# BenLangmead/bowtie2

Measured on NVIDIA H100. Metric: Mreads/s, higher is better.
Workload: dtype u64 popcount (FM rank) + s16x2 DPX (DP)

## Files before the change

bowtie2_b200/csrc/dp_kernels.cu:

```cuda
#include "fm_device.cuh"
#include "dp_device.cuh"

#define DP_NEG (-(1 << 28))
#define DP_BIG (1 << 20)

__host__ __device__ __forceinline__ size_t dp_smem_per_warp(int maxCol) { return ((size_t)maxCol * 7 + 16 + 15) & ~(size_t)15; }

__device__ __forceinline__ int dp_max(int a, int b) { return a > b ? a : b; }

template <int R>
__device__ __forceinline__ void dp_backtrace_all(const DpLaunch &L, const bt2g_scoring &sc, const bt2g_dp_problem &p, uint64_t w,
                                                 const uint8_t *rs, const uint8_t *rq, int rdlen, const uint8_t *refw,
                                                 uint8_t *codes, bt2g_dp_cand *cands, int ncand, bt2g_dp_summary *summ,
                                                 int lane, bool local) {
	const int rdgapo = sc.rdgap_const + sc.rdgap_linear, rdgape = sc.rdgap_linear;
	const int rfgapo = sc.rfgap_const + sc.rfgap_linear, rfgape = sc.rfgap_linear;
	int SQ = rdlen >> 4; if(SQ == 0) SQ = 1;
	bt2g_dp_aln *alns = L.alns + w * (uint64_t)L.maxAlns;
	uint8_t *ops = L.ops + w * (uint64_t)L.maxAlns * L.maxOps;
	int naln = 0, flags = 0;
	auto cell = [&](int rr, int cc) -> uint8_t * { int k = rr / R; return codes + ((size_t)(cc + k) * 32 + k) * R + (rr - k * R); };
	for(int ci = 0; ci < ncand; ci++) {
		int row = cands[ci].row, col = cands[ci].col;
		const int startRow = row;
// ... 79 lines not shown
			const int c = rdchar(row), refc = refw[col];
			const bool isN = c > 3 || refc > 3;
			ns += isN;
			const uint8_t op = (uint8_t)(((!isN && c == refc) ? BT2G_OP_MATCH : BT2G_OP_MM) | (refc << 2));
			if(!core) fail = true;
			else if(ns > p.nceil) fail = true;
			else {
				if(room && lane == 0 && nops < L.maxOps) o[nops] = op;
				nops++;
			}
		}
		const bool opOverflow = nops > L.maxOps;
		if(fail) { if(lane == 0) cands[ci].fate = BT2G_CAND_FAILED; continue; }
		if(lane == 0) cands[ci].fate = BT2G_CAND_SUCCEEDED;
		if(room) {
			int refns = 0;
			for(int k = col + lane; k <= origCol; k += 32) refns += refw[k] > 3;
			refns = __reduce_add_sync(0xffffffffu, refns);
			if(lane == 0) {
				bt2g_dp_aln &a = alns[naln];
				a.cand_idx = ci; a.score = cands[ci].score; a.ns = ns; a.gaps = gaps; a.col0 = col; a.row0 = row;
				a.trim_beg = trimBeg; a.trim_end = rdlen - 1 - startRow; a.nops = nops;
				a.refns = refns;
			}
			if(opOverflow) flags |= BT2G_DP_FLAG_OPS_OVERFLOW;
		} else {
			flags |= BT2G_DP_FLAG_ALN_OVERFLOW;
		}
		naln++;
	}
	if(lane == 0) { summ->naln = naln; summ->flags |= flags; }
}

template <typename Acc>
__device__ __forceinline__ void dp_backtrace_h(const DpLaunch &L, const bt2g_scoring &sc, const bt2g_dp_problem &p, uint64_t w,
                                               const uint8_t *rs, const uint8_t *rq, int rdlen, const uint8_t *refw,
                                               const Acc &cell, bt2g_dp_cand *cands, int ncand, bt2g_dp_summary *summ, int lane,
                                               const uint8_t *prof);

template <int R, bool HB = false, typename Acc = int>
__device__ __forceinline__ void dp_e2e_tail(const DpLaunch &L, const bt2g_scoring &sc, const bt2g_dp_problem &p, uint64_t w,
                                            const uint8_t *rs, const uint8_t *rq, int rdlen, int ncol, int32_t *lastH,
                                            uint16_t *candCol, const uint8_t *refw, uint8_t *codes, bt2g_dp_summary *summ, int lane,
                                            const Acc &hcell = Acc(), const uint8_t *prof = nullptr) {
	__syncwarp();
	int best = DP_NEG;
	for(int k = lane; k < ncol; k += 32) best = dp_max(best, lastH[k]);
#pragma unroll
	for(int o = 16; o > 0; o >>= 1) best = dp_max(best, __shfl_xor_sync(0xffffffffu, best, o));

	if(lane == 0) { summ->best = best; summ->flags = 0; summ->naln = 0; summ->ncand = 0; summ->found = 0; }
	if(best < p.minsc) return;
	bt2g_dp_cand *cands = L.cands + w * (uint64_t)L.maxCands;
	int totalCand = 0;
	for(int j0 = 0; j0 < ncol; j0 += 32) {
		const int j = j0 + lane;
		const int s = j < ncol ? lastH[j] : DP_NEG;
		const bool isC = j < ncol && s >= p.minsc;
		const uint32_t m = __ballot_sync(0xffffffffu, isC);
		if(isC) {
			const int k = totalCand + __popc(m & ((1u << lane) - 1u));
			lastH[k] = s; candCol[k] = (uint16_t)j;
		}
		totalCand += __popc(m);
		__syncwarp();
	}
	for(int a0 = 0; a0 < totalCand; a0 += 32) {
		const int a = a0 + lane;
		if(a < totalCand) {
			const int s = lastH[a];
			int rank = 0;
			for(int k = 0; k < totalCand; k++) {
				const int sk = lastH[k];
				rank += (sk > s) || (sk == s && k > a);
			}
			if(rank < L.maxCands) { cands[rank].score = s; cands[rank].col = candCol[a]; cands[rank].row = rdlen - 1; cands[rank].fate = 0; }
		}
	}
	const int ncand = totalCand < L.maxCands ? totalCand : L.maxCands;
	if(lane == 0) {
		summ->ncand = totalCand; summ->found = totalCand > 0;
		if(totalCand > L.maxCands) summ->flags |= BT2G_DP_FLAG_CAND_OVERFLOW;
	}
	__syncwarp();

	if constexpr(HB) dp_backtrace_h(L, sc, p, w, rs, rq, rdlen, refw, hcell, cands, ncand, summ, lane, prof);
	else dp_backtrace_all<R>(L, sc, p, w, rs, rq, rdlen, refw, codes, cands, ncand, summ, lane, false);
}

template <typename OFF, int R>
__global__ void __launch_bounds__(128) k_dp_e2e(DevIndex<OFF> ix, bt2g_scoring sc, DpLaunch L) {
	extern __shared__ uint8_t smem[];
	const int warpInBlock = threadIdx.x >> 5, lane = threadIdx.x & 31;
	const uint64_t slot = blockIdx.x * (uint64_t)(blockDim.x >> 5) + warpInBlock;
	const uint64_t nSlots = (uint64_t)gridDim.x * (blockDim.x >> 5);
	const uint64_t nProb = L.nDev ? (uint64_t)*L.nDev : L.n;
	const size_t perWarp = dp_smem_per_warp(L.maxCol);
	int32_t *lastH = reinterpret_cast<int32_t *>(smem + (size_t)warpInBlock * perWarp);
	uint16_t *candCol = reinterpret_cast<uint16_t *>(lastH + L.maxCol);
	uint8_t *refw = reinterpret_cast<uint8_t *>(candCol + L.maxCol);
	uint8_t *codes = L.codes + slot * L.codeStride;
	const int rdgapo = sc.rdgap_const + sc.rdgap_linear, rdgape = sc.rdgap_linear;
	const int rfgapo = sc.rfgap_const + sc.rfgap_linear, rfgape = sc.rfgap_linear;

	for(uint64_t w = slot; w < nProb; w += nSlots) {
		const bt2g_dp_problem p = L.probs[w];
		const uint8_t *rs = L.seq + L.roff[p.read_idx];
		const uint8_t *rq = L.qual + L.roff[p.read_idx];
		const int rdlen = (int)(L.roff[p.read_idx + 1] - L.roff[p.read_idx]);
		const int ncol = (int)(p.refr - p.refl + 1);
		bt2g_dp_summary *summ = L.summ + w;
		__syncwarp();
		if(ncol <= 0 || ncol > L.maxCol || rdlen > 32 * R || rdlen <= 0) {
			if(lane == 0) { summ->found = 0; summ->best = DP_NEG; summ->ncand = 0; summ->naln = 0; summ->flags = BT2G_DP_FLAG_BADSHAPE; }
			continue;
		}
		for(int k = lane; k < ncol; k += 32) refw[k] = (uint8_t)ref_base<OFF>(ix, p.tidx, p.refl + k);
		__syncwarp();

		int rc[R], mmpN[R], npnN[R], rfo[R], rfe[R], rdo[R];
// ... 607 lines not shown
						if(!TOP && OFFDOM && lo + t0 + SG - 1 >= bLast) {
							uint32_t s = botH | botF | prevInH;
#pragma unroll
							for(int r = 0; r < RPL; r++) s |= Hleft[r] | Earr[r];
							if(!__any_sync(0xffffffffu, t0 + SG - 1 - lane < lim && s != 0u)) return t0 + SG < nsteps ? t0 + SG : nsteps;
						}
					}
					return nsteps;
				};
				nst = b == 0 ? sweep(DpBool<true>()) : sweep(DpBool<false>());
			}
			if(lane == 0) {
				reinterpret_cast<uint32_t *>(hb[0])[b] = (uint32_t)lo | ((uint32_t)nst << 16);
				reinterpret_cast<uint32_t *>(hb[1])[b] = (uint32_t)lo | ((uint32_t)nst << 16);
			}
			off += (uint32_t)nst * 32 * RPL;
			plo = lo; phi = lo + nst - 32;
			if(phi > ncolMax - 1) phi = ncolMax - 1;
			__syncwarp();
		}
	}
}

struct DpHbBlocks {
	uint8_t *hb; const uint2 *tab;
	__device__ __forceinline__ uint8_t *operator()(int rr, int cc) const {
		const int k = (rr % DP_BLK_ROWS) / DP_BLOCK_RPL;
		const uint2 e = tab[rr / DP_BLK_ROWS];
		const int st = cc - (int)(e.x & 0xffffu) + k;
		return (st >= k && st < (int)(e.x >> 16)) ? hb + e.y + ((size_t)st * 32 + k) * DP_BLOCK_RPL + rr % DP_BLOCK_RPL : nullptr;
	}
};

#define DP_TAIL_SMEM_PER_WARP(maxCol, R) (dp_smem_per_warp(maxCol) + DP_PROF_BYTES(R) + DP_BLK_MAX * sizeof(uint2))

template <typename OFF, int R>
__global__ void __launch_bounds__(256) k_dp_tail_h(DevIndex<OFF> ix, bt2g_scoring sc, DpLaunch L, uint64_t chunkStart, uint64_t chunkMax,
                                                   uint32_t *next) {
	extern __shared__ uint8_t smem[];
	const int warpInBlock = threadIdx.x >> 5, lane = threadIdx.x & 31;
	const uint64_t nAll = L.nDev ? (uint64_t)*L.nDev : L.n;
	if(chunkStart >= nAll) return;
	const uint64_t nProb = (nAll - chunkStart < chunkMax) ? nAll - chunkStart : chunkMax;
	const size_t perWarp = DP_TAIL_SMEM_PER_WARP(L.maxCol, R);
	int32_t *lastH = reinterpret_cast<int32_t *>(smem + (size_t)warpInBlock * perWarp);
	uint16_t *candCol = reinterpret_cast<uint16_t *>(lastH + L.maxCol);
	uint8_t *refw = reinterpret_cast<uint8_t *>(candCol + L.maxCol);
	uint8_t *prof = smem + (size_t)warpInBlock * perWarp + dp_smem_per_warp(L.maxCol);
	uint2 *tab = reinterpret_cast<uint2 *>(prof + DP_PROF_BYTES(R));
	const int bonus = sc.match_bonus;
	for(uint64_t wl = dp_next_task(next, lane); wl < nProb; wl = dp_next_task(next, lane)) {
		const uint64_t w = chunkStart + wl;
		const bt2g_dp_problem p = L.probs[w];
		const uint8_t *rs = L.seq + L.roff[p.read_idx], *rq = L.qual + L.roff[p.read_idx];
		const int rdlen = (int)(L.roff[p.read_idx + 1] - L.roff[p.read_idx]);
		const int ncol = (int)(p.refr - p.refl + 1);
		const int floorv = p.minsc - bonus - 1;
		__syncwarp();
		if(ncol <= 0 || ncol > L.maxCol || rdlen > 32 * R || rdlen <= 0 || (int64_t)bonus * rdlen - floorv > 127 || floorv < -DPX_LIMIT) continue;
		uint8_t *hb = L.codes + wl * L.codeStride;
		const int nblk = (rdlen + DP_BLK_ROWS - 1) / DP_BLK_ROWS;
		const uint32_t e = lane < nblk ? reinterpret_cast<const uint32_t *>(hb)[lane] : 0u;
		const uint32_t bytes = (e >> 16) * (32 * DP_BLOCK_RPL);
		uint32_t incl = bytes;
#pragma unroll
		for(int o = 1; o < 32; o <<= 1) { const uint32_t v = __shfl_up_sync(0xffffffffu, incl, o); if(lane >= o) incl += v; }
		if(lane < nblk) tab[lane] = make_uint2(e, DP_BLK_HEAD + incl - bytes);
		ref_window<OFF>(ix, p.tidx, p.refl, ncol, refw, lane);
		for(int i = lane; i < rdlen; i += 32) {
			const int pos = p.fw ? i : rdlen - 1 - i;
			int c = rs[pos]; c = p.fw ? c : (c > 3 ? 4 : 3 - c);
			int q = (int)rq[pos] - 33; q = q < 0 ? 0 : (q > 63 ? 63 : q);
			prof[i] = (uint8_t)c; prof[rdlen + i] = sc.mmpen[q]; prof[2 * rdlen + i] = sc.npen[q];
		}
		__syncwarp();
		const DpHbBlocks cell{hb, tab};
		const int lr = rdlen - 1;
		for(int j = lane; j < ncol; j += 32) { const uint8_t *c = cell(lr, j); lastH[j] = (c ? (int)*c : 0) + floorv; }
		dp_e2e_tail<R, true>(L, sc, p, w, rs, rq, rdlen, ncol, lastH, candCol, refw, hb, L.summ + w, lane, cell, prof);
	}
}

template <typename Acc>
__device__ __forceinline__ void dp_backtrace_h(const DpLaunch &L, const bt2g_scoring &sc, const bt2g_dp_problem &p, uint64_t w,
                                               const uint8_t *rs, const uint8_t *rq, int rdlen, const uint8_t *refw,
                                               const Acc &cell, bt2g_dp_cand *cands, int ncand, bt2g_dp_summary *summ, int lane,
                                               const uint8_t *prof) {
	const int rdgapo = sc.rdgap_const + sc.rdgap_linear, rdgape = sc.rdgap_linear;
	const int rfgapo = sc.rfgap_const + sc.rfgap_linear, rfgape = sc.rfgap_linear;
	const int bonus = sc.match_bonus, gapbar = sc.gapbar;
	const int vmax = bonus * rdlen - (p.minsc - bonus - 1);
	bt2g_dp_aln *alns = L.alns + w * (uint64_t)L.maxAlns;
	uint8_t *ops = L.ops + w * (uint64_t)L.maxAlns * L.maxOps;
	int naln = 0, flags = 0;
	bool screened = false;
	auto cellv = [&](int rr, int cc) -> int { const uint8_t *c = cell(rr, cc); return c ? (int)*c : 0; };
	auto rdchar = [&](int rr) -> int { const int pos = p.fw ? rr : rdlen - 1 - rr; int c = rs[pos]; return p.fw ? c : (c > 3 ? 4 : 3 - c); };
	auto rdqual = [&](int rr) -> int { const int pos = p.fw ? rr : rdlen - 1 - rr; int q = (int)rq[pos] - 33; return q < 0 ? 0 : (q > 63 ? 63 : q); };
	auto inCore = [&](int dlo, int dhi) -> bool { return dhi >= p.corel && dlo <= p.corer; };
	for(int ci = 0; ci < ncand; ci++) {
		int row = cands[ci].row, col = cands[ci].col;
		const int startRow = row, origCol = col;
		uint8_t *o = ops + (size_t)naln * L.maxOps;
		const bool room = naln < L.maxAlns;
		int nops = 0, ns = 0, gaps = 0;
		bool fail = false, core = false, done = false, first = true, filtStart = false;
		while(!done && !fail) {
			const int wd = (ci > 0 && first) ? 8 : 32;
			const int rk = row - lane, ck = col - lane;
			const bool in = lane < wd && rk >= 0 && ck >= 0;
			uint8_t *cp = in ? cell(rk, ck) : nullptr;
			const int mine = in ? (cp ? (int)*cp : 0) : 0x80;
			const int v = mine & 0x7f;
			const int vn = __shfl_down_sync(0xffffffffu, v, 1);
			int sck = 0, refc = 4; bool isN = false, isMatch = false;
			if(in) {
				refc = refw[ck];
				if(prof) {
					const int c = prof[rk];
					isN = c > 3 || refc > 3;
					isMatch = !isN && c == refc;
					sck = isN ? -(int)prof[2 * rdlen + rk] : (isMatch ? bonus : -(int)prof[rdlen + rk]);
				} else {
					const int c = rdchar(rk), q = rdqual(rk);
					isN = c > 3 || refc > 3;
					isMatch = !isN && c == refc;
					sck = isN ? -(int)sc.npen[q] : (isMatch ? bonus : -(int)sc.mmpen[q]);
				}
			}
			const bool cont = lane < wd - 1 && !(mine & 0x80) && rk > 0 && ck > 0 && vn > 0 && v == vn + sck;
			const int run = __ffs(~__ballot_sync(0xffffffffu, cont)) - 1;
			if(run > 0) {
				first = false;
				const int diagi = col - row + p.triml;
				if(inCore(diagi, diagi)) core = true;
				if(lane < run) {
					const uint8_t op = (uint8_t)((isMatch ? BT2G_OP_MATCH : BT2G_OP_MM) | (refc << 2));
					if(room && nops + lane < L.maxOps) o[nops + lane] = op;
					if(cp) *cp = (uint8_t)(mine | 0x80);
				}
				ns += __popc(__ballot_sync(0xffffffffu, lane < run && isN));
				nops += run; row -= run; col -= run;
			}
			const int endBits = __shfl_sync(0xffffffffu, mine, run);
			if(run == wd - 1 && !(endBits & 0x80) && row > 0 && col > 0) { __syncwarp(); continue; }
			if(endBits & 0x80) {
				if(first) filtStart = true;
				fail = true; break;
			}
			first = false;
			if(lane == run && cp) *cp = (uint8_t)(mine | 0x80);
			{
				const int diagi = col - row + p.triml;
				if(inCore(diagi, diagi)) core = true;
			}
			if(row == 0) { done = true; break; }
			const int cur = endBits & 0x7f;
			__syncwarp();
			int klen = 0, gapKind = 0;
			if(row >= gapbar && rdlen - 1 - row >= gapbar) {
				for(int k0 = 0; k0 < row; k0 += 32) {
					if(vmax - rfgapo - k0 * rfgape < cur) break;
					const int k = k0 + lane + 1, r2 = row - k;
					bool ok = false;
					if(r2 >= 0 && row - k + 1 >= gapbar && vmax - rfgapo - (k - 1) * rfgape >= cur) {
						const int u = cellv(r2, col) & 0x7f;
						ok = u > 0 && u - rfgapo - (k - 1) * rfgape == cur;
					}
					const uint32_t mk = __ballot_sync(0xffffffffu, ok);
					if(mk) { klen = k0 + __ffs(mk); gapKind = 1; break; }
				}
				if(gapKind == 0) {
					for(int k0 = 0; k0 < col; k0 += 32) {
						if(vmax - rdgapo - k0 * rdgape < cur) break;
						const int k = k0 + lane + 1, c2 = col - k;
						bool ok = false;
						if(c2 >= 0 && vmax - rdgapo - (k - 1) * rdgape >= cur) {
							const int u = cellv(row, c2) & 0x7f;
							ok = u > 0 && u - rdgapo - (k - 1) * rdgape == cur;
						}
						const uint32_t mk = __ballot_sync(0xffffffffu, ok);
						if(mk) { klen = k0 + __ffs(mk); gapKind = 2; break; }
					}
				}
			}
			if(gapKind == 0) { fail = true; break; }
			for(int m0 = 1; m0 < klen && !fail; m0 += 32) {
				const int mth = m0 + lane;
				uint8_t *q2 = nullptr; int b = 0;
				if(mth < klen) { q2 = gapKind == 1 ? cell(row - mth, col) : cell(row, col - mth); b = q2 ? *q2 : 0; }
				const uint32_t vm = __ballot_sync(0xffffffffu, (b & 0x80) != 0);
				const int lim = vm ? __ffs(vm) - 1 : 32;
				if(q2 && lane < lim) *q2 = (uint8_t)(b | 0x80);
				if(vm) fail = true;
			}
			if(fail) break;
			{
				const int d0 = col - row + p.triml, ni = klen - 1;
				if(ni > 0 && (gapKind == 1 ? inCore(d0 + 1, d0 + ni) : inCore(d0 - ni, d0 - 1))) core = true;
			}
			if(room) {
				for(int k = lane; k < klen; k += 32) {
					const int idx = nops + k;
					if(idx < L.maxOps) o[idx] = gapKind == 1 ? (uint8_t)BT2G_OP_REFGAP : (uint8_t)(BT2G_OP_READGAP | (refw[col - k] << 2));
				}
			}
			nops += klen; gaps += klen;
			if(gapKind == 1) row -= klen; else col -= klen;
			__syncwarp();
		}
		if(filtStart) { if(lane == 0) cands[ci].fate = BT2G_CAND_FILT_START; continue; }
		if(!fail) {
			const int c = rdchar(row), refc = refw[col];
			const bool isN = c > 3 || refc > 3;
			ns += isN;
			const uint8_t op = (uint8_t)(((!isN && c == refc) ? BT2G_OP_MATCH : BT2G_OP_MM) | (refc << 2));
			if(!core) fail = true;
			else if(ns > p.nceil) fail = true;
			else {
				if(room && lane == 0 && nops < L.maxOps) o[nops] = op;
				nops++;
			}
		}
		const bool opOverflow = nops > L.maxOps;
		if(fail) { if(lane == 0) cands[ci].fate = BT2G_CAND_FAILED; continue; }
		if(lane == 0) cands[ci].fate = BT2G_CAND_SUCCEEDED;
		if(room) {
			int refns = 0;
			for(int k = col + lane; k <= origCol; k += 32) refns += refw[k] > 3;
			refns = __reduce_add_sync(0xffffffffu, refns);
			if(lane == 0) {
				bt2g_dp_aln &a = alns[naln];
				a.cand_idx = ci; a.score = cands[ci].score; a.ns = ns; a.gaps = gaps; a.col0 = col; a.row0 = row;
				a.trim_beg = 0; a.trim_end = rdlen - 1 - startRow; a.nops = nops;
				a.refns = refns;
			}
			if(opOverflow) flags |= BT2G_DP_FLAG_OPS_OVERFLOW;
		} else {
			flags |= BT2G_DP_FLAG_ALN_OVERFLOW;
		}
		naln++;
		if(naln == 1 && !screened && ci + 1 < ncand) {
			screened = true;
			bool needSeq = false;
			for(int base = ci + 1; base < ncand; base += 32) {
				const int cj = base + lane;
				int verdict = 0;
				if(cj < ncand) {
					int r2 = cands[cj].row, c2 = cands[cj].col;
					int b = cellv(r2, c2);
					if(b & 0x80) verdict = 1;
					else {
						for(int guard = 0; guard < 4 * rdlen + 8; guard++) {
							const int curv = b & 0x7f;
							if(r2 == 0) { verdict = 2; break; }
							if(c2 > 0) {
								const int pb = cellv(r2 - 1, c2 - 1), pv = pb & 0x7f;
								const int rf = refw[c2];
								int c, mm, np;
								if(prof) { c = prof[r2]; mm = prof[rdlen + r2]; np = prof[2 * rdlen + r2]; }
								else { c = rdchar(r2); const int q = rdqual(r2); mm = sc.mmpen[q]; np = sc.npen[q]; }
								const int sc2 = (c > 3 || rf > 3) ? -np : (c == rf ? bonus : -mm);
								if(pv > 0 && curv == pv + sc2) {
									if(pb & 0x80) break;
									r2--; c2--; b = pb;
									continue;
								}
							}
							if(r2 < gapbar || rdlen - 1 - r2 < gapbar) break;
							bool moved = false, dead = false, marked = false;
							for(int k = 1; k <= r2 && r2 - k + 1 >= gapbar && vmax - rfgapo - (k - 1) * rfgape >= curv; k++) {
								const int ub = cellv(r2 - k, c2), u = ub & 0x7f;
								if(u > 0 && u - rfgapo - (k - 1) * rfgape == curv) {
									if(marked || (ub & 0x80)) dead = true; else { r2 -= k; b = ub; moved = true; }
									break;
								}
								marked = marked || (ub & 0x80);
							}
							if(!moved && !dead) {
								marked = false;
								for(int k = 1; k <= c2 && vmax - rdgapo - (k - 1) * rdgape >= curv; k++) {
									const int ub = cellv(r2, c2 - k), u = ub & 0x7f;
									if(u > 0 && u - rdgapo - (k - 1) * rdgape == curv) {
										if(marked || (ub & 0x80)) dead = true; else { c2 -= k; b = ub; moved = true; }
										break;
									}
									marked = marked || (ub & 0x80);
								}
							}
							if(!moved) break;
						}
					}
				}
				if(__any_sync(0xffffffffu, verdict == 2)) { needSeq = true; break; }
				if(cj < ncand) cands[cj].fate = verdict == 1 ? BT2G_CAND_FILT_START : BT2G_CAND_FAILED;
			}
			__syncwarp();
			if(!needSeq) break;
		}
	}
	if(lane == 0) { summ->naln = naln; summ->flags |= flags; }
}

template <typename K>
static unsigned dp_resident_grid(K kernel, int threads, size_t smem, uint64_t numSlots, int warpsPerBlock) {
	int dev = 0, sms = 148, nb = 1;
	cudaGetDevice(&dev);
	cudaDeviceGetAttribute(&sms, cudaDevAttrMultiProcessorCount, dev);
	if(cudaOccupancyMaxActiveBlocksPerMultiprocessor(&nb, kernel, threads, smem) != cudaSuccess || nb < 1) nb = 1;
	uint64_t g = (uint64_t)nb * sms, cap = numSlots / warpsPerBlock;
	return (unsigned)(g < cap ? g : cap);
}

template <typename K>
static int dp_block_warps(K kernel, size_t perWarp, int want, size_t *smem) {
	int dev = 0, optin = 48 * 1024;
	cudaGetDevice(&dev);
	if(cudaDeviceGetAttribute(&optin, cudaDevAttrMaxSharedMemoryPerBlockOptin, dev) != cudaSuccess) return 0;
	cudaFuncAttributes fa;
	if(cudaFuncGetAttributes(&fa, kernel) != cudaSuccess) return 0;
	const size_t room = (size_t)optin > fa.sharedSizeBytes ? (size_t)optin - fa.sharedSizeBytes : 0;
	int w = want;
	while(w > 1 && (size_t)w * perWarp > room) w--;
	if((size_t)w * perWarp > room) return 0;
	*smem = (size_t)w * perWarp;
	if(*smem > 48 * 1024 && cudaFuncSetAttribute(kernel, cudaFuncAttributeMaxDynamicSharedMemorySize, (int)*smem) != cudaSuccess) return 0;
	return w;
}

template <typename OFF, int R>
static int launch_dp_e2e_r(const DevIndex<OFF> &ix, const bt2g_scoring &sc, const DpLaunch &L, cudaStream_t st) {
	if(L.packed == 3) {
		if(!L.taskCtr) return -1;
		int dev = 0, sms = 148; cudaGetDevice(&dev); cudaDeviceGetAttribute(&sms, cudaDevAttrMultiProcessorCount, dev);
// ... 236 lines not shown
```

bowtie2_b200/csrc/xengine.cuh:

```cuda
#pragma once
#include <stdint.h>
#include "../../include/bt2g.h"
#include "mapq_device.cuh"
#include "pe_device.cuh"

#ifndef XE_HD
#define XE_HD __host__ __device__
#endif
#define XE_HH __host__ __device__

namespace xe {

#define XE_MIN_I64 (-9223372036854775807LL - 1)
#define XE_BIG ((int64_t)1 << 62)
enum { EXHAUSTED = 1, FULFILLED, PERFECT, SOFT_LIMIT, HARD_LIMIT };
enum { XR_DONE = 0, XR_ONE_MM = 1, XR_SEED = 2, XR_DP = 3, XR_DP_MATE = 4, XR_FALLBACK = 5 };

#define XE_MAX_LEN    512
#define XE_ARENA      12288
#define XE_SEEN_IV    224
#define XE_EXR        8
#define XE_MM1        24
#define XE_MAX_SEEDS  64
#define XE_SATS       (2 * XE_MAX_SEEDS)
// ... 48 lines not shown
	XE_HD uint64_t u64() { const uint64_t hi = u32(); return (hi << 32) | u32(); }
	XE_HD int boolean() { if(lastOff > 31) u32(); const int r = (last >> lastOff) & 1; lastOff++; return r; }
	XE_HD double flt() { return (double)((float)u32() / (float)0xffffffff); }
};

struct XEdit { int16_t pos; uint8_t chr, qchr, type, pad; };
struct XAln {
	int64_t refoff; int32_t tidx, score; int16_t rdlen, trim5, trim3, nedits; uint8_t fw, ns, refns, pad;
	XE_HD XEdit *edits() { return reinterpret_cast<XEdit *>(this + 1); }
	XE_HD const XEdit *edits() const { return reinterpret_cast<const XEdit *>(this + 1); }
	XE_HD int ext() const { return rdlen - trim5 - trim3; }
	XE_HD int trimLeft() const { return fw ? trim5 : trim3; }
	XE_HD int refExtent() const { int e = ext(); const XEdit *ed = edits(); for(int i = 0; i < nedits; i++) e += (ed[i].type == 1) - (ed[i].type == 2); return e; }
};

struct XEEHit { uint64_t top, bot; int32_t score; int16_t pos; uint8_t fw, hasEdit, chr, qchr, pad[2];
	XE_HD int ns() const { return hasEdit && (chr == 'N' || qchr == 'N'); }
	XE_HD int refns() const { return hasEdit && chr == 'N'; } };

struct XIv { int64_t a; int32_t tidx, len; };
struct XExr { int32_t p5, len; int64_t size; };

struct XRand {
	uint32_t n, cur, thresh; uint16_t listOff; uint8_t swaplist, converted;
};
struct XSeen { uint32_t val; uint16_t owner, pad; };

struct XSat { uint64_t topf, topb; int64_t size; int16_t rdoff, seedlen; uint8_t fw, offidx, nlex, nrex; uint8_t rix, elim, pad[2]; double mass; };
struct XEnt { uint64_t topf; int32_t size; int16_t rdoff, seedlen; uint8_t fw; int8_t ee; uint8_t rix, done1, mateStreak, pad[3]; };

struct XMate {
	int32_t idx, rdlen, nceil; int64_t minsc, perfect;
	uint8_t filt, nee, nmm1, hasSh; uint8_t nexr[2]; uint16_t nseen;
	XEEHit ee[2], mm1[XE_MM1];
	XExr exr[2][XE_EXR];
	XIv seen[XE_SEEN_IV];
	int32_t shN, shInterval, shOffset, shSeedlen; int64_t shNonz, shNelt;
	uint16_t nranks; uint8_t ranks[2 * XE_MAX_SEEDS];
};

struct XDpReq { bt2g_dp_problem prob; };

struct XUnit {
	int32_t pc, pcExt; uint8_t fallback, paired, doneFlag, pad0;
	uint32_t id;
	XRng rnd;
	XMate m[2]; int32_t cur;
	int64_t khits, mhits;
	uint8_t doneConcord, doneDiscord, doneUnp[2], exitConcordM, exitConcordK, psDone, pad1;
	int64_t nconcord, nunp[2], bestPair, best2Pair;
	uint16_t nrs12, nrs1u, nrs2u; uint16_t rs1[XE_LIST], rs2[XE_LIST], rs1u[XE_LIST], rs2u[XE_LIST];
	uint8_t usDone, usExitM, usExitK, pad2; int64_t usBest, usBest2; uint16_t nus; uint16_t usAlns[XE_LIST];
	uint16_t nred[3]; uint16_t red[3][XE_RED];
	uint32_t redKey[3][XE_RED];
	int64_t nIters, nDps, nUgs, nMateDps, streakCur;
	int32_t interval[2], nrounds[2], matemap[2], mi, roundi, nroundsAll; int64_t nelt[2]; int32_t mined[2][2];
	uint8_t done[2], nofwM[2], norcM[2], both, rdone;
	int32_t xAi, xUseSh, xUseEe, xRet;
	uint8_t eeMode, firstEe, firstExtend, swMateImmediately;
	int64_t nEeFail, nUgFail, nDpFail, neltLeft, streak, nonz;
	int32_t si, nents; XEnt ents[XE_ENTS];
	int32_t nsats; XSat sats[XE_SATS];
	int32_t nrands; XRand rands[XE_RANDS];
	int32_t nseenPool; XSeen seenPool[XE_SEENPOOL];
	int32_t nhitl; XEEHit hitl[XE_HITL];
	uint8_t isSmall, fw, first, state, firstInner, foundConcordant, foundMate, didAnchor, brk, haveOa, oleft, ofw, dpU8, odpU8, pad3[2];
	int32_t rdoff, readGaps, refGaps;
	int64_t tidx, toff, tlen, refoff, ominscCur;
	uint16_t fixedAln, curAln;
	int32_t natt, attCursor; int16_t attScore[XE_ATT]; uint16_t attAln[XE_ATT];
	int32_t mateCursor, mateAlnK;
	bt2g_dp_problem rqProb;
	int32_t rqRead, rqMinsc, rqNofw, rqNorc, rqL, rqInterval, rqOffset;
	int32_t dpSlot;
	int32_t pairType, pairKind; int64_t scoreSum, fraglen;
	uint8_t resAligned[2], resHasXs[2]; int32_t resMapq[2]; int64_t resXs[2]; uint16_t resAln[2];
	uint32_t arenaTop; uint32_t fbLine;
	alignas(8) uint8_t arena[XE_ARENA];
};

XE_HD inline XAln *x_aln(XUnit &u, uint16_t off) { return reinterpret_cast<XAln *>(u.arena + (size_t)off * 8); }
XE_HD inline const XAln *x_aln(const XUnit &u, uint16_t off) { return reinterpret_cast<const XAln *>(u.arena + (size_t)off * 8); }
XE_HD inline uint16_t x_alloc(XUnit &u, uint32_t bytes) {
	const uint32_t need = (bytes + 7u) & ~7u;
	if(u.arenaTop + need > XE_ARENA) { XE_FB(u); return 0xffff; }
	const uint16_t off = (uint16_t)(u.arenaTop >> 3);
	u.arenaTop += need;
	return off;
}
XE_HD inline uint16_t x_new_aln(XUnit &u, int nedits) {
	const uint16_t off = x_alloc(u, (uint32_t)(sizeof(XAln) + (size_t)nedits * sizeof(XEdit)));
	if(off == 0xffff) return off;
	XAln *a = x_aln(u, off);
	a->refoff = 0; a->tidx = 0; a->score = 0; a->rdlen = 0; a->trim5 = a->trim3 = 0; a->nedits = (int16_t)nedits; a->fw = 1; a->ns = a->refns = a->pad = 0;
	return off;
}

XE_HD inline char x_dna(int c) { return c == 0 ? 'A' : c == 1 ? 'C' : c == 2 ? 'G' : c == 3 ? 'T' : 'N'; }
XE_HD inline int x_code(int ch) { return ch == 'A' ? 0 : ch == 'C' ? 1 : ch == 'G' ? 2 : ch == 'T' ? 3 : 4; }
XE_HD inline int x_rdchar(const uint8_t *codes, int rdlen, bool fw, int row) {
	if(fw) return codes[row];
	const int c = codes[rdlen - 1 - row];
	return c > 3 ? 4 : 3 - c;
}

XE_HD inline uint16_t *x_rlist(XUnit &u, const XRand &r) { return reinterpret_cast<uint16_t *>(u.arena + (size_t)r.listOff * 8); }
XE_HD inline void x_rand_init(XUnit &u, XRand &r, uint64_t n, bool all) {
	r.n = (uint32_t)n; r.cur = 0; r.converted = 0; r.swaplist = (n < 128 || all) ? 1 : 0; r.listOff = 0xffff;
	const uint32_t t = (uint32_t)(0.10f * (float)n);
	r.thresh = t > 16 ? t : 16;
// ... 41 lines not shown
			for(int i = 0; i < u.nseenPool; i++) if(u.seenPool[i].owner == (uint16_t)rix && u.seenPool[i].val == j) { s = true; break; }
			if(!s) l[k++] = (uint16_t)j;
		}
		int w = 0;
		for(int i = 0; i < u.nseenPool; i++) if(u.seenPool[i].owner != (uint16_t)rix) u.seenPool[w++] = u.seenPool[i];
		u.nseenPool = w;
		r.cur = 0; r.n = rest; r.converted = 1; r.swaplist = 1;
	}
	return rn;
}
XE_HD inline int x_new_rand(XUnit &u, uint64_t n, bool all) {
	if(u.nrands >= XE_RANDS) { XE_FB(u); return 0; }
	const int rix = u.nrands++;
	x_rand_init(u, u.rands[rix], n, all);
	return rix;
}

template <typename T>
XE_HD inline void x_shuffle_portion(T *v, int begin, int num, XRng &rnd) {
	if(num < 2) return;
	int left = num;
	for(int i = begin; i < begin + num - 1; i++) {
		const int r = (int)(rnd.u64() % (uint64_t)left);
		if(r > 0) { const T t = v[i]; v[i] = v[i + r]; v[i + r] = t; }
		left--;
	}
}

XE_HD inline void x_seen_add(XUnit &u, XMate &c, int64_t tidx, bool fw, int64_t off, int64_t len) {
	if(c.nseen >= XE_SEEN_IV) { XE_FB(u); return; }
	XIv &x = c.seen[c.nseen++];
	x.a = off; x.len = (int32_t)len; x.tidx = (int32_t)((uint32_t)tidx | (fw ? 0x80000000u : 0u));
}
XE_HD inline bool x_seen_present(const XMate &c, int64_t tidx, bool fw, int64_t off) {
	const int32_t key = (int32_t)((uint32_t)tidx | (fw ? 0x80000000u : 0u));
	for(int i = 0; i < c.nseen; i++) { const XIv &x = c.seen[i]; if(x.tidx == key && x.a <= off && off < x.a + x.len) return true; }
	return false;
}

struct XCellIt {
	const XAln *a; const XEdit *ed; int k, i, n; int64_t left, right, diff;
	XE_HD void init(const XAln *al) { a = al; ed = al->edits(); k = 0; i = al->trimLeft(); n = i + al->ext(); left = al->refoff; right = left + 1; diff = 1; fetch(); }
	XE_HD bool valid() const { return i < n; }
	XE_HD void fetch() {
		if(i >= n) return;
		diff = 1; right = left + 1;
		const int rel = i - a->trimLeft();
		while(k < a->nedits && ed[k].pos == rel) { if(ed[k].type == 2) diff = 0; k++; }
		if(i < n - 1) { int k2 = k; while(k2 < a->nedits && ed[k2].pos == rel + 1) { if(ed[k2].type == 1) right++; k2++; } }
	}
	XE_HD void next() { left = right + diff - 1; i++; fetch(); }
};
XE_HD inline bool x_alns_share_cell(const XAln *a, const XAln *b) {
	if(a->tidx != b->tidx || a->fw != b->fw) return false;
	const int64_t d = a->refoff - b->refoff;
	if(d > 1200 || d < -1200) return false;
	XCellIt x, y; x.init(a); y.init(b);
	while(x.valid() && y.valid()) {
		if(x.i < y.i) { x.next(); continue; }
		if(y.i < x.i) { y.next(); continue; }
		if(x.left < y.right && y.left < x.right) return true;
		x.next(); y.next();
	}
	return false;
}
XE_HD inline uint32_t x_red_key(const XAln *a) {
	return (((uint32_t)a->tidx * 2u + (uint32_t)(a->fw != 0)) << 20) | ((uint32_t)((uint64_t)a->refoff >> 11) & 0xfffffu);
}
XE_HD inline bool x_red_overlap(const XUnit &u, int set, uint16_t aoff) {
	const XAln *a = x_aln(u, aoff);
	const uint32_t ka = x_red_key(a);
	for(int i = 0; i < u.nred[set]; i++) {
		const uint32_t kb = u.redKey[set][i];
		if((ka ^ kb) >> 20) continue;
		if(((kb - ka + 1u) & 0xfffffu) > 2u) continue;
		if(x_alns_share_cell(a, x_aln(u, u.red[set][i]))) return true;
	}
	return false;
}
XE_HD inline void x_red_add(XUnit &u, int set, uint16_t aoff) {
	if(u.nred[set] >= XE_RED) { XE_FB(u); return; }
	u.redKey[set][u.nred[set]] = x_red_key(x_aln(u, aoff));
	u.red[set][u.nred[set]++] = aoff;
}

struct XRect { int64_t refl, refr, reflPre, refrPre, triml, trimr, corel, corer, maxgap; };
XE_HD inline bool x_frame_seed(int64_t off, int rdlen, int64_t reflen, int maxrdgap, int maxrfgap, int maxhalf, XRect &r) {
	const uint64_t a = (uint64_t)(int64_t)maxrdgap, b = (uint64_t)(int64_t)maxrfgap;
	const uint64_t mx = a > b ? a : b;
	const int64_t maxgap = (int64_t)(mx < (uint64_t)maxhalf ? mx : (uint64_t)maxhalf);
	const int64_t refl = off - 2 * maxgap, refr = off + (rdlen - 1) + 2 * maxgap;
	int64_t triml = 0, trimr = 0;
	if(refr >= reflen) trimr = refr - (reflen - 1);
	if(refl < 0) triml = -refl;
	r.refl = refl + triml; r.refr = refr - trimr; r.reflPre = refl; r.refrPre = refr; r.triml = triml; r.trimr = trimr;
	r.corel = maxgap; r.corer = maxgap + 2 * maxgap; r.maxgap = maxgap;
	return !(r.refr < r.refl);
}
XE_HD inline bool x_frame_mate(bool anchorLeft, int64_t ll, int64_t lr, int64_t rl, int64_t rr, int rdlen, int64_t reflen, int maxrdgap, int maxrfgap,
                               int maxhalf, XRect &r) {
	const uint64_t a = (uint64_t)(int64_t)maxrdgap, b = (uint64_t)(int64_t)maxrfgap;
	uint64_t mx = a > b ? a : b; if((uint64_t)maxhalf > mx) mx = (uint64_t)maxhalf;
	const int64_t maxgap = (int64_t)mx;
	int64_t refl, refr;
	if(anchorLeft) { refl = (rl - (rdlen - 1)) - maxgap; refr = rr + maxgap; }
	else { refl = ll - maxgap; refr = (lr + (rdlen - 1)) + maxgap; }
	int64_t triml = 0, trimr = 0;
	if(refr >= reflen) trimr = refr - (reflen - 1);
	if(refl < 0) triml = -refl;
// ... 1128 lines not shown
```

Before: 2.786.

## Early-exit DP tail before ref window/profile; store last row as bytes; prune gap scans

The tail kernel now reads the last H row as raw 8-bit values, computes the best score, and skips problems below the minimum score before fetching the reference window and building the read profile. The last-row buffer shrinks from int32 to uint8, with the score offset applied inside a new shared candidate routine. The block-table load is hoisted ahead of the problem read, and the screening backtrace skips gap scans when the adjacent cell already bounds them out. Optional compile-time profiling probes are added, but they compile to no-ops by default.

```diff
diff --git a/bowtie2_b200/csrc/dp_kernels.cu b/bowtie2_b200/csrc/dp_kernels.cu
--- a/bowtie2_b200/csrc/dp_kernels.cu
+++ b/bowtie2_b200/csrc/dp_kernels.cu
@@ -135,11 +135,122 @@
 	if(lane == 0) { summ->naln = naln; summ->flags |= flags; }
 }
 
+enum { DPT_FETCH, DPT_WINDOW, DPT_PROFILE, DPT_LASTROW, DPT_RANK, DPT_FIRST_BT, DPT_SCREEN, DPT_SEQ, DPT_NPHASE };
+#define DPT_NHIST 8
+#ifdef BT2G_DP_TAIL_PROFILE
+struct DpTailProfRec {
+	unsigned long long key, warps, probs, nobest, clk[DPT_NPHASE], hist[DPT_NHIST], rounds, gapIters, gapCells;
+	unsigned long long scrGroups, scrStepsMax, scrStepsSum, scrGapMax, scrGapSum;
+};
+#define DPT_NREC 4
+__device__ DpTailProfRec g_dpTailProf[DPT_NREC];
+struct DpTailProbe {
+	long long t = 0;
+	unsigned long long clk[DPT_NPHASE] = {}, hist[DPT_NHIST] = {}, probs = 0, nobest = 0, rounds = 0, gapIters = 0, gapCells = 0;
+	unsigned long long scrGroups = 0, scrStepsMax = 0, scrStepsSum = 0, scrGapMax = 0, scrGapSum = 0;
+	__device__ __forceinline__ void start() { t = clock64(); }
+	__device__ __forceinline__ void phase(int k) { __syncwarp(); const long long n = clock64(); clk[k] += (unsigned long long)(n - t); t = n; }
+	__device__ __forceinline__ void problem(int ncand) {
+		probs++; nobest += ncand == 0;
+		const int b = ncand == 0 ? 0 : (32 - __clz(ncand) < DPT_NHIST - 1 ? 32 - __clz(ncand) : DPT_NHIST - 1);
+#pragma unroll
+		for(int i = 0; i < DPT_NHIST; i++) hist[i] += i == b;
+	}
+	__device__ __forceinline__ void round() { rounds++; }
+	__device__ __forceinline__ void gapIter() { gapIters++; }
+	__device__ __forceinline__ void gapCell(int n) { gapCells += n; }
+	__device__ __forceinline__ void screen(int steps, int gap) {
+		scrGroups++;
+		scrStepsMax += __reduce_max_sync(0xffffffffu, (unsigned)steps); scrStepsSum += __reduce_add_sync(0xffffffffu, (unsigned)steps);
+		scrGapMax += __reduce_max_sync(0xffffffffu, (unsigned)gap); scrGapSum += __reduce_add_sync(0xffffffffu, (unsigned)gap);
+	}
+	__device__ void flush(unsigned long long key, int lane) {
+		if(lane != 0) return;
+		int s = 0;
+		for(; s < DPT_NREC - 1; s++) {
+			const unsigned long long k = atomicCAS(&g_dpTailProf[s].key, 0ull, key);
+			if(k == 0 || k == key) break;
+		}
+		DpTailProfRec &r = g_dpTailProf[s];
+		atomicAdd(&r.warps, 1ull); atomicAdd(&r.probs, probs); atomicAdd(&r.nobest, nobest);
+#pragma unroll
+		for(int i = 0; i < DPT_NPHASE; i++) atomicAdd(&r.clk[i], clk[i]);
+#pragma unroll
+		for(int i = 0; i < DPT_NHIST; i++) atomicAdd(&r.hist[i], hist[i]);
+		atomicAdd(&r.rounds, rounds); atomicAdd(&r.gapIters, gapIters); atomicAdd(&r.gapCells, gapCells);
+		atomicAdd(&r.scrGroups, scrGroups); atomicAdd(&r.scrStepsMax, scrStepsMax); atomicAdd(&r.scrStepsSum, scrStepsSum);
+		atomicAdd(&r.scrGapMax, scrGapMax); atomicAdd(&r.scrGapSum, scrGapSum);
+	}
+};
+extern "C" int bt2g_dp_tail_profile(unsigned long long *out, int reset) {
+	if(out && cudaMemcpyFromSymbol(out, g_dpTailProf, sizeof(g_dpTailProf)) != cudaSuccess) return -1;
+	if(reset) {
+		static const DpTailProfRec zero[DPT_NREC] = {};
+		if(cudaMemcpyToSymbol(g_dpTailProf, zero, sizeof(g_dpTailProf)) != cudaSuccess) return -1;
+	}
+	return (int)(sizeof(g_dpTailProf) / sizeof(unsigned long long));
+}
+#else
+struct DpTailProbe {
+	__device__ __forceinline__ void start() {}
+	__device__ __forceinline__ void phase(int) {}
+	__device__ __forceinline__ void problem(int) {}
+	__device__ __forceinline__ void round() {}
+	__device__ __forceinline__ void gapIter() {}
+	__device__ __forceinline__ void gapCell(int) {}
+	__device__ __forceinline__ void screen(int, int) {}
+	__device__ __forceinline__ void flush(unsigned long long, int) {}
+};
+#endif
+
 template <typename Acc>
 __device__ __forceinline__ void dp_backtrace_h(const DpLaunch &L, const bt2g_scoring &sc, const bt2g_dp_problem &p, uint64_t w,
                                                const uint8_t *rs, const uint8_t *rq, int rdlen, const uint8_t *refw,
                                                const Acc &cell, bt2g_dp_cand *cands, int ncand, bt2g_dp_summary *summ, int lane,
-                                               const uint8_t *prof);
+                                               const uint8_t *prof, DpTailProbe *pr = nullptr);
+
+template <int R, bool HB = false, typename Acc = int, typename T = int32_t>
+__device__ __forceinline__ void dp_e2e_cands(const DpLaunch &L, const bt2g_scoring &sc, const bt2g_dp_problem &p, uint64_t w,
+                                             const uint8_t *rs, const uint8_t *rq, int rdlen, int ncol, T *lastH, int sOff,
+                                             uint16_t *candCol, const uint8_t *refw, uint8_t *codes, bt2g_dp_summary *summ, int lane,
+                                             const Acc &hcell = Acc(), const uint8_t *prof = nullptr, DpTailProbe *pr = nullptr) {
+	bt2g_dp_cand *cands = L.cands + w * (uint64_t)L.maxCands;
+	int totalCand = 0;
+	for(int j0 = 0; j0 < ncol; j0 += 32) {
+		const int j = j0 + lane;
+		const T v = j < ncol ? lastH[j] : T(0);
+		const bool isC = j < ncol && (int)v + sOff >= p.minsc;
+		const uint32_t m = __ballot_sync(0xffffffffu, isC);
+		if(isC) {
+			const int k = totalCand + __popc(m & ((1u << lane) - 1u));
+			lastH[k] = v; candCol[k] = (uint16_t)j;
+		}
+		totalCand += __popc(m);
+		__syncwarp();
+	}
+	for(int a0 = 0; a0 < totalCand; a0 += 32) {
+		const int a = a0 + lane;
+		if(a < totalCand) {
+			const int s = lastH[a];
+			int rank = 0;
+			for(int k = 0; k < totalCand; k++) {
+				const int sk = lastH[k];
+				rank += (sk > s) || (sk == s && k > a);
+			}
+			if(rank < L.maxCands) { cands[rank].score = s + sOff; cands[rank].col = candCol[a]; cands[rank].row = rdlen - 1; cands[rank].fate = 0; }
+		}
+	}
+	const int ncand = totalCand < L.maxCands ? totalCand : L.maxCands;
+	if(lane == 0) {
+		summ->ncand = totalCand; summ->found = totalCand > 0;
+		if(totalCand > L.maxCands) summ->flags |= BT2G_DP_FLAG_CAND_OVERFLOW;
+	}
+	__syncwarp();
+	if(pr) { pr->problem(totalCand); pr->phase(DPT_RANK); }
+
+	if constexpr(HB) dp_backtrace_h(L, sc, p, w, rs, rq, rdlen, refw, hcell, cands, ncand, summ, lane, prof, pr);
+	else dp_backtrace_all<R>(L, sc, p, w, rs, rq, rdlen, refw, codes, cands, ncand, summ, lane, false);
+}
 
 template <int R, bool HB = false, typename Acc = int>
 __device__ __forceinline__ void dp_e2e_tail(const DpLaunch &L, const bt2g_scoring &sc, const bt2g_dp_problem &p, uint64_t w,
@@ -154,41 +265,7 @@
 
 	if(lane == 0) { summ->best = best; summ->flags = 0; summ->naln = 0; summ->ncand = 0; summ->found = 0; }
 	if(best < p.minsc) return;
-	bt2g_dp_cand *cands = L.cands + w * (uint64_t)L.maxCands;
-	int totalCand = 0;
-	for(int j0 = 0; j0 < ncol; j0 += 32) {
-		const int j = j0 + lane;
-		const int s = j < ncol ? lastH[j] : DP_NEG;
-		const bool isC = j < ncol && s >= p.minsc;
-		const uint32_t m = __ballot_sync(0xffffffffu, isC);
-		if(isC) {
-			const int k = totalCand + __popc(m & ((1u << lane) - 1u));
-			lastH[k] = s; candCol[k] = (uint16_t)j;
-		}
-		totalCand += __popc(m);
-		__syncwarp();
-	}
-	for(int a0 = 0; a0 < totalCand; a0 += 32) {
-		const int a = a0 + lane;
-		if(a < totalCand) {
-			const int s = lastH[a];
-			int rank = 0;
-			for(int k = 0; k < totalCand; k++) {
-				const int sk = lastH[k];
-				rank += (sk > s) || (sk == s && k > a);
-			}
-			if(rank < L.maxCands) { cands[rank].score = s; cands[rank].col = candCol[a]; cands[rank].row = rdlen - 1; cands[rank].fate = 0; }
-		}
-	}
-	const int ncand = totalCand < L.maxCands ? totalCand : L.maxCands;
-	if(lane == 0) {
-		summ->ncand = totalCand; summ->found = totalCand > 0;
-		if(totalCand > L.maxCands) summ->flags |= BT2G_DP_FLAG_CAND_OVERFLOW;
-	}
-	__syncwarp();
-
-	if constexpr(HB) dp_backtrace_h(L, sc, p, w, rs, rq, rdlen, refw, hcell, cands, ncand, summ, lane, prof);
-	else dp_backtrace_all<R>(L, sc, p, w, rs, rq, rdlen, refw, codes, cands, ncand, summ, lane, false);
+	dp_e2e_cands<R, HB>(L, sc, p, w, rs, rq, rdlen, ncol, lastH, 0, candCol, refw, codes, summ, lane, hcell, prof);
 }
 
 template <typename OFF, int R>
@@ -862,7 +939,8 @@
 	}
 };
 
-#define DP_TAIL_SMEM_PER_WARP(maxCol, R) (dp_smem_per_warp(maxCol) + DP_PROF_BYTES(R) + DP_BLK_MAX * sizeof(uint2))
+__host__ __device__ __forceinline__ size_t dp_tail_prof_off(int maxCol) { return ((size_t)DP_BLK_MAX * sizeof(uint2) + (size_t)maxCol * 4 + 16 + 15) & ~(size_t)15; }
+#define DP_TAIL_SMEM_PER_WARP(maxCol, R) (dp_tail_prof_off(maxCol) + DP_PROF_BYTES(R))
 
 template <typename OFF, int R>
 __global__ void __launch_bounds__(256) k_dp_tail_h(DevIndex<OFF> ix, bt2g_scoring sc, DpLaunch L, uint64_t chunkStart, uint64_t chunkMax,
@@ -872,31 +950,51 @@
 	const uint64_t nAll = L.nDev ? (uint64_t)*L.nDev : L.n;
 	if(chunkStart >= nAll) return;
 	const uint64_t nProb = (nAll - chunkStart < chunkMax) ? nAll - chunkStart : chunkMax;
-	const size_t perWarp = DP_TAIL_SMEM_PER_WARP(L.maxCol, R);
-	int32_t *lastH = reinterpret_cast<int32_t *>(smem + (size_t)warpInBlock * perWarp);
-	uint16_t *candCol = reinterpret_cast<uint16_t *>(lastH + L.maxCol);
-	uint8_t *refw = reinterpret_cast<uint8_t *>(candCol + L.maxCol);
-	uint8_t *prof = smem + (size_t)warpInBlock * perWarp + dp_smem_per_warp(L.maxCol);
-	uint2 *tab = reinterpret_cast<uint2 *>(prof + DP_PROF_BYTES(R));
+	uint8_t *sw = smem + (size_t)warpInBlock * DP_TAIL_SMEM_PER_WARP(L.maxCol, R);
+	uint2 *tab = reinterpret_cast<uint2 *>(sw);
+	uint16_t *candCol = reinterpret_cast<uint16_t *>(sw + DP_BLK_MAX * sizeof(uint2));
+	uint8_t *lastH = reinterpret_cast<uint8_t *>(candCol + L.maxCol);
+	uint8_t *refw = lastH + L.maxCol;
+	uint8_t *prof = sw + dp_tail_prof_off(L.maxCol);
 	const int bonus = sc.match_bonus;
+	DpTailProbe pr;
+	pr.start();
 	for(uint64_t wl = dp_next_task(next, lane); wl < nProb; wl = dp_next_task(next, lane)) {
 		const uint64_t w = chunkStart + wl;
+		uint8_t *hb = L.codes + wl * L.codeStride;
+		const uint32_t e0 = lane < DP_BLK_MAX ? reinterpret_cast<const uint32_t *>(hb)[lane] : 0u;
 		const bt2g_dp_problem p = L.probs[w];
-		const uint8_t *rs = L.seq + L.roff[p.read_idx], *rq = L.qual + L.roff[p.read_idx];
-		const int rdlen = (int)(L.roff[p.read_idx + 1] - L.roff[p.read_idx]);
+		const uint64_t ro = L.roff[p.read_idx];
+		const int rdlen = (int)(L.roff[p.read_idx + 1] - ro);
+		const uint8_t *rs = L.seq + ro, *rq = L.qual + ro;
 		const int ncol = (int)(p.refr - p.refl + 1);
 		const int floorv = p.minsc - bonus - 1;
 		__syncwarp();
 		if(ncol <= 0 || ncol > L.maxCol || rdlen > 32 * R || rdlen <= 0 || (int64_t)bonus * rdlen - floorv > 127 || floorv < -DPX_LIMIT) continue;
-		uint8_t *hb = L.codes + wl * L.codeStride;
 		const int nblk = (rdlen + DP_BLK_ROWS - 1) / DP_BLK_ROWS;
-		const uint32_t e = lane < nblk ? reinterpret_cast<const uint32_t *>(hb)[lane] : 0u;
+		const uint32_t e = lane < nblk ? e0 : 0u;
 		const uint32_t bytes = (e >> 16) * (32 * DP_BLOCK_RPL);
 		uint32_t incl = bytes;
 #pragma unroll
 		for(int o = 1; o < 32; o <<= 1) { const uint32_t v = __shfl_up_sync(0xffffffffu, incl, o); if(lane >= o) incl += v; }
 		if(lane < nblk) tab[lane] = make_uint2(e, DP_BLK_HEAD + incl - bytes);
+		__syncwarp();
+		pr.phase(DPT_FETCH);
+		const DpHbBlocks cell{hb, tab};
+		const int lr = rdlen - 1;
+		int mx = 0;
+		for(int j = lane; j < ncol; j += 32) {
+			const uint8_t *c = cell(lr, j);
+			const int v = c ? (int)*c : 0;
+			lastH[j] = (uint8_t)v; mx = dp_max(mx, v);
+		}
+		const int best = (int)__reduce_max_sync(0xffffffffu, (unsigned)mx) + floorv;
+		bt2g_dp_summary *summ = L.summ + w;
+		if(lane == 0) { summ->best = best; summ->flags = 0; summ->naln = 0; summ->ncand = 0; summ->found = 0; }
+		pr.phase(DPT_LASTROW);
+		if(best < p.minsc) { pr.problem(0); continue; }
 		ref_window<OFF>(ix, p.tidx, p.refl, ncol, refw, lane);
+		pr.phase(DPT_WINDOW);
 		for(int i = lane; i < rdlen; i += 32) {
 			const int pos = p.fw ? i : rdlen - 1 - i;
 			int c = rs[pos]; c = p.fw ? c : (c > 3 ? 4 : 3 - c);
@@ -904,22 +1002,23 @@
 			prof[i] = (uint8_t)c; prof[rdlen + i] = sc.mmpen[q]; prof[2 * rdlen + i] = sc.npen[q];
 		}
 		__syncwarp();
-		const DpHbBlocks cell{hb, tab};
-		const int lr = rdlen - 1;
-		for(int j = lane; j < ncol; j += 32) { const uint8_t *c = cell(lr, j); lastH[j] = (c ? (int)*c : 0) + floorv; }
-		dp_e2e_tail<R, true>(L, sc, p, w, rs, rq, rdlen, ncol, lastH, candCol, refw, hb, L.summ + w, lane, cell, prof);
-	}
+		pr.phase(DPT_PROFILE);
+		dp_e2e_cands<R, true>(L, sc, p, w, rs, rq, rdlen, ncol, lastH, floorv, candCol, refw, hb, summ, lane, cell, prof, &pr);
+	}
+	pr.phase(DPT_FETCH);
+	pr.flush(L.maxCol, lane);
 }
 
 template <typename Acc>
 __device__ __forceinline__ void dp_backtrace_h(const DpLaunch &L, const bt2g_scoring &sc, const bt2g_dp_problem &p, uint64_t w,
                                                const uint8_t *rs, const uint8_t *rq, int rdlen, const uint8_t *refw,
                                                const Acc &cell, bt2g_dp_cand *cands, int ncand, bt2g_dp_summary *summ, int lane,
-                                               const uint8_t *prof) {
+                                               const uint8_t *prof, DpTailProbe *pr) {
 	const int rdgapo = sc.rdgap_const + sc.rdgap_linear, rdgape = sc.rdgap_linear;
 	const int rfgapo = sc.rfgap_const + sc.rfgap_linear, rfgape = sc.rfgap_linear;
 	const int bonus = sc.match_bonus, gapbar = sc.gapbar;
 	const int vmax = bonus * rdlen - (p.minsc - bonus - 1);
+	const bool rfBound = rfgapo >= rfgape, rdBound = rdgapo >= rdgape;
 	bt2g_dp_aln *alns = L.alns + w * (uint64_t)L.maxAlns;
 	uint8_t *ops = L.ops + w * (uint64_t)L.maxAlns * L.maxOps;
 	int naln = 0, flags = 0;
@@ -936,6 +1035,7 @@
 		int nops = 0, ns = 0, gaps = 0;
 		bool fail = false, core = false, done = false, first = true, filtStart = false;
 		while(!done && !fail) {
+			if(pr) pr->round();
 			const int wd = (ci > 0 && first) ? 8 : 32;
 			const int rk = row - lane, ck = col - lane;
 			const bool in = lane < wd && rk >= 0 && ck >= 0;
@@ -991,6 +1091,7 @@
 			if(row >= gapbar && rdlen - 1 - row >= gapbar) {
 				for(int k0 = 0; k0 < row; k0 += 32) {
 					if(vmax - rfgapo - k0 * rfgape < cur) break;
+					if(pr) pr->gapIter();
 					const int k = k0 + lane + 1, r2 = row - k;
 					bool ok = false;
 					if(r2 >= 0 && row - k + 1 >= gapbar && vmax - rfgapo - (k - 1) * rfgape >= cur) {
@@ -1003,6 +1104,7 @@
 				if(gapKind == 0) {
 					for(int k0 = 0; k0 < col; k0 += 32) {
 						if(vmax - rdgapo - k0 * rdgape < cur) break;
+						if(pr) pr->gapIter();
 						const int k = k0 + lane + 1, c2 = col - k;
 						bool ok = false;
 						if(c2 >= 0 && vmax - rdgapo - (k - 1) * rdgape >= cur) {
@@ -1015,6 +1117,7 @@
 				}
 			}
 			if(gapKind == 0) { fail = true; break; }
+			if(pr) pr->gapCell(klen - 1);
 			for(int m0 = 1; m0 < klen && !fail; m0 += 32) {
 				const int mth = m0 + lane;
 				uint8_t *q2 = nullptr; int b = 0;
@@ -1072,16 +1175,19 @@
 		naln++;
 		if(naln == 1 && !screened && ci + 1 < ncand) {
 			screened = true;
+			if(pr) pr->phase(DPT_FIRST_BT);
 			bool needSeq = false;
 			for(int base = ci + 1; base < ncand; base += 32) {
 				const int cj = base + lane;
 				int verdict = 0;
+				int nSteps = 0, nGap = 0;
 				if(cj < ncand) {
 					int r2 = cands[cj].row, c2 = cands[cj].col;
 					int b = cellv(r2, c2);
 					if(b & 0x80) verdict = 1;
 					else {
 						for(int guard = 0; guard < 4 * rdlen + 8; guard++) {
+							nSteps++;
 							const int curv = b & 0x7f;
 							if(r2 == 0) { verdict = 2; break; }
 							if(c2 > 0) {
@@ -1099,7 +1205,9 @@
 							}
 							if(r2 < gapbar || rdlen - 1 - r2 < gapbar) break;
 							bool moved = false, dead = false, marked = false;
-							for(int k = 1; k <= r2 && r2 - k + 1 >= gapbar && vmax - rfgapo - (k - 1) * rfgape >= curv; k++) {
+							const bool rfScan = !rfBound || (cellv(r2 - 1, c2) & 0x7f) - rfgape >= curv;
+							for(int k = 1; rfScan && k <= r2 && r2 - k + 1 >= gapbar && vmax - rfgapo - (k - 1) * rfgape >= curv; k++) {
+								nGap++;
 								const int ub = cellv(r2 - k, c2), u = ub & 0x7f;
 								if(u > 0 && u - rfgapo - (k - 1) * rfgape == curv) {
 									if(marked || (ub & 0x80)) dead = true; else { r2 -= k; b = ub; moved = true; }
@@ -1107,9 +1215,10 @@
 								}
 								marked = marked || (ub & 0x80);
 							}
-							if(!moved && !dead) {
+							if(!moved && !dead && c2 > 0 && (!rdBound || (cellv(r2, c2 - 1) & 0x7f) - rdgape >= curv)) {
 								marked = false;
 								for(int k = 1; k <= c2 && vmax - rdgapo - (k - 1) * rdgape >= curv; k++) {
+									nGap++;
 									const int ub = cellv(r2, c2 - k), u = ub & 0x7f;
 									if(u > 0 && u - rdgapo - (k - 1) * rdgape == curv) {
 										if(marked || (ub & 0x80)) dead = true; else { c2 -= k; b = ub; moved = true; }
@@ -1122,14 +1231,17 @@
 						}
 					}
 				}
+				if(pr) pr->screen(nSteps, nGap);
 				if(__any_sync(0xffffffffu, verdict == 2)) { needSeq = true; break; }
 				if(cj < ncand) cands[cj].fate = verdict == 1 ? BT2G_CAND_FILT_START : BT2G_CAND_FAILED;
 			}
 			__syncwarp();
+			if(pr) pr->phase(DPT_SCREEN);
 			if(!needSeq) break;
 		}
 	}
 	if(lane == 0) { summ->naln = naln; summ->flags |= flags; }
+	if(pr) pr->phase(screened ? DPT_SEQ : DPT_FIRST_BT);
 }
 
 template <typename K>
```

Result: faster. 2.850 (median of 6 runs) (+2.3%).

## Move scalar fields ahead of arrays in XUnit and batch-load linear scans

Applied to the files above, without the earlier changes.

Reorders the XUnit and XMate structs so scalar counters and small fields are grouped together ahead of the large arrays. This is meant to improve locality of the frequently touched state (likely in local or global memory per thread). The seen-interval and redundancy-key scans now load groups of eight entries at once so the loads can be issued back to back before they are compared. The grouped loads may read stale slots past the valid count, which are masked out, and they add register pressure.

```diff
diff --git a/bowtie2_b200/csrc/xengine.cuh b/bowtie2_b200/csrc/xengine.cuh
--- a/bowtie2_b200/csrc/xengine.cuh
+++ b/bowtie2_b200/csrc/xengine.cuh
@@ -104,11 +104,11 @@
 struct XMate {
 	int32_t idx, rdlen, nceil; int64_t minsc, perfect;
 	uint8_t filt, nee, nmm1, hasSh; uint8_t nexr[2]; uint16_t nseen;
+	int32_t shN, shInterval, shOffset, shSeedlen; int64_t shNonz, shNelt;
+	uint16_t nranks; uint8_t ranks[2 * XE_MAX_SEEDS];
 	XEEHit ee[2], mm1[XE_MM1];
 	XExr exr[2][XE_EXR];
 	XIv seen[XE_SEEN_IV];
-	int32_t shN, shInterval, shOffset, shSeedlen; int64_t shNonz, shNelt;
-	uint16_t nranks; uint8_t ranks[2 * XE_MAX_SEEDS];
 };
 
 struct XDpReq { bt2g_dp_problem prob; };
@@ -117,30 +117,25 @@
 	int32_t pc, pcExt; uint8_t fallback, paired, doneFlag, pad0;
 	uint32_t id;
 	XRng rnd;
-	XMate m[2]; int32_t cur;
+	int32_t cur;
 	int64_t khits, mhits;
 	uint8_t doneConcord, doneDiscord, doneUnp[2], exitConcordM, exitConcordK, psDone, pad1;
 	int64_t nconcord, nunp[2], bestPair, best2Pair;
-	uint16_t nrs12, nrs1u, nrs2u; uint16_t rs1[XE_LIST], rs2[XE_LIST], rs1u[XE_LIST], rs2u[XE_LIST];
-	uint8_t usDone, usExitM, usExitK, pad2; int64_t usBest, usBest2; uint16_t nus; uint16_t usAlns[XE_LIST];
-	uint16_t nred[3]; uint16_t red[3][XE_RED];
-	uint32_t redKey[3][XE_RED];
+	uint16_t nrs12, nrs1u, nrs2u;
+	uint8_t usDone, usExitM, usExitK, pad2; int64_t usBest, usBest2; uint16_t nus;
+	uint16_t nred[3];
 	int64_t nIters, nDps, nUgs, nMateDps, streakCur;
 	int32_t interval[2], nrounds[2], matemap[2], mi, roundi, nroundsAll; int64_t nelt[2]; int32_t mined[2][2];
 	uint8_t done[2], nofwM[2], norcM[2], both, rdone;
 	int32_t xAi, xUseSh, xUseEe, xRet;
 	uint8_t eeMode, firstEe, firstExtend, swMateImmediately;
 	int64_t nEeFail, nUgFail, nDpFail, neltLeft, streak, nonz;
-	int32_t si, nents; XEnt ents[XE_ENTS];
-	int32_t nsats; XSat sats[XE_SATS];
-	int32_t nrands; XRand rands[XE_RANDS];
-	int32_t nseenPool; XSeen seenPool[XE_SEENPOOL];
-	int32_t nhitl; XEEHit hitl[XE_HITL];
+	int32_t si, nents, nsats, nrands, nseenPool, nhitl;
 	uint8_t isSmall, fw, first, state, firstInner, foundConcordant, foundMate, didAnchor, brk, haveOa, oleft, ofw, dpU8, odpU8, pad3[2];
 	int32_t rdoff, readGaps, refGaps;
 	int64_t tidx, toff, tlen, refoff, ominscCur;
 	uint16_t fixedAln, curAln;
-	int32_t natt, attCursor; int16_t attScore[XE_ATT]; uint16_t attAln[XE_ATT];
+	int32_t natt, attCursor;
 	int32_t mateCursor, mateAlnK;
 	bt2g_dp_problem rqProb;
 	int32_t rqRead, rqMinsc, rqNofw, rqNorc, rqL, rqInterval, rqOffset;
@@ -148,6 +143,17 @@
 	int32_t pairType, pairKind; int64_t scoreSum, fraglen;
 	uint8_t resAligned[2], resHasXs[2]; int32_t resMapq[2]; int64_t resXs[2]; uint16_t resAln[2];
 	uint32_t arenaTop; uint32_t fbLine;
+	XMate m[2];
+	uint16_t rs1[XE_LIST], rs2[XE_LIST], rs1u[XE_LIST], rs2u[XE_LIST];
+	uint16_t usAlns[XE_LIST];
+	uint32_t redKey[3][XE_RED];
+	uint16_t red[3][XE_RED];
+	int16_t attScore[XE_ATT]; uint16_t attAln[XE_ATT];
+	XEEHit hitl[XE_HITL];
+	XEnt ents[XE_ENTS];
+	XSat sats[XE_SATS];
+	XRand rands[XE_RANDS];
+	XSeen seenPool[XE_SEENPOOL];
 	alignas(8) uint8_t arena[XE_ARENA];
 };
 
@@ -255,9 +261,18 @@
 	XIv &x = c.seen[c.nseen++];
 	x.a = off; x.len = (int32_t)len; x.tidx = (int32_t)((uint32_t)tidx | (fw ? 0x80000000u : 0u));
 }
+#define XE_SCAN_GROUP 8
+static_assert(XE_SEEN_IV % XE_SCAN_GROUP == 0 && XE_RED % XE_SCAN_GROUP == 0, "scan groups stay inside the arrays");
 XE_HD inline bool x_seen_present(const XMate &c, int64_t tidx, bool fw, int64_t off) {
 	const int32_t key = (int32_t)((uint32_t)tidx | (fw ? 0x80000000u : 0u));
-	for(int i = 0; i < c.nseen; i++) { const XIv &x = c.seen[i]; if(x.tidx == key && x.a <= off && off < x.a + x.len) return true; }
+	const int n = c.nseen;
+	for(int i = 0; i < n; i += XE_SCAN_GROUP) {
+		XIv x[XE_SCAN_GROUP];
+		for(int k = 0; k < XE_SCAN_GROUP; k++) x[k] = c.seen[i + k];
+		bool hit = false;
+		for(int k = 0; k < XE_SCAN_GROUP; k++) hit |= i + k < n && x[k].tidx == key && x[k].a <= off && off < x[k].a + x[k].len;
+		if(hit) return true;
+	}
 	return false;
 }
 
@@ -293,11 +308,16 @@
 XE_HD inline bool x_red_overlap(const XUnit &u, int set, uint16_t aoff) {
 	const XAln *a = x_aln(u, aoff);
 	const uint32_t ka = x_red_key(a);
-	for(int i = 0; i < u.nred[set]; i++) {
-		const uint32_t kb = u.redKey[set][i];
-		if((ka ^ kb) >> 20) continue;
-		if(((kb - ka + 1u) & 0xfffffu) > 2u) continue;
-		if(x_alns_share_cell(a, x_aln(u, u.red[set][i]))) return true;
+	const int n = u.nred[set];
+	for(int i0 = 0; i0 < n; i0 += XE_SCAN_GROUP) {
+		uint32_t kg[XE_SCAN_GROUP];
+		for(int k = 0; k < XE_SCAN_GROUP; k++) kg[k] = u.redKey[set][i0 + k];
+		for(int k = 0; k < XE_SCAN_GROUP && i0 + k < n; k++) {
+			const uint32_t kb = kg[k];
+			if((ka ^ kb) >> 20) continue;
+			if(((kb - ka + 1u) & 0xfffffu) > 2u) continue;
+			if(x_alns_share_cell(a, x_aln(u, u.red[set][i0 + k]))) return true;
+		}
 	}
 	return false;
 }
```

Result: faster. 2.792 before, 2.946 after (median of 6 runs) (+5.5%).
